# eldariont/svim

Measured on AMD Instinct MI355X. Metric: aligned reads/sec through COLLECT+CLUSTER, higher is better.
Workload: dtype u32/i32 CIGAR + u8 bases, int64 positions, f64 distances

## Files before the change

include/svx.h:

```cpp
#ifndef SVX_H
#define SVX_H
#include <stdint.h>
#ifdef __cplusplus
extern "C" {
#endif

#define SVX_OK               0
#define SVX_E_NODEVICE     (-1)
#define SVX_E_HIP          (-2)
#define SVX_E_ARG          (-3)
#define SVX_E_CAPACITY     (-4)
#define SVX_E_STATE        (-5)
#define SVX_E_FASTA_SYMBOL (-6)
#define SVX_E_FASTA_HOST   (-7)
#define SVX_E_NO_DELETION  (-8)

enum { SVX_DEL = 0, SVX_INS = 1, SVX_INV = 2, SVX_DUP_TAN = 3, SVX_BND = 4, SVX_DUP_INT = 5, SVX_NTYPES = 6 };
enum { SVX_SRC_CIGAR = 0, SVX_SRC_SUPPL = 1 };
enum { SVX_LEFT_FWD = 0, SVX_LEFT_REV = 1, SVX_RIGHT_FWD = 2, SVX_RIGHT_REV = 3, SVX_DIR_ALL = 4 };

#define SVX_FLAG_SKIP 0x8000u
#define SVX_FLAG_SA   0x4000u

typedef struct svx_params {
// ... 27 lines not shown
    const uint32_t* seg_off;
    int64_t n_seg;
    const int32_t*  seg_tid;
    const int32_t*  seg_pos;
    const uint8_t*  seg_rev;
    const uint8_t*  seg_mapq;
    const int32_t*  seg_lseq;
    const uint64_t* seg_cigar_off;
    const uint32_t* seg_cigar;
    int32_t n_contig;
    const int32_t*  contig_rank;
    const uint32_t* seq_rng_off;
    const int32_t*  seq_rng_q0;
    const int32_t*  seq_rng_len;
    const uint64_t* seq_rng_byte;
    int64_t n_seq_rng;
} svx_batch;

typedef struct svx_sig_view {
    int32_t on_device;
    int64_t n;
    uint64_t* key;
    uint8_t*  type;
    uint8_t*  src;
    uint8_t*  aux;
    int32_t*  contig;
    int32_t*  start;
    int32_t*  end;
    int32_t*  contig2;
    int32_t*  pos2;
    int32_t*  read_id;
    int64_t*  seq_off;
    uint8_t*  seq;
} svx_sig_view;

typedef struct svx_genome {
    int32_t on_device;
    int32_t n_contig;
    const int64_t* off;
    const uint8_t* codes;
} svx_genome;

typedef struct svx_cluster_view {
    int64_t n;
    int64_t type_count[SVX_NTYPES];
    uint8_t* type;
    int32_t* contig;  int32_t* start;  int32_t* end;
    int32_t* contig2; int32_t* start2; int32_t* end2;
    uint8_t* aux;
    double*  score;
    double*  std_span;
    double*  std_pos;
    int32_t* size;
    int64_t* member_off;
    int32_t* members;
    int64_t  n_members;
} svx_cluster_view;

typedef struct svx_ctx svx_ctx;

typedef struct svx_stats {
    double  t_collect_ms, t_cluster_ms;
    double  t_cigar_scan_ms, t_segments_ms, t_sort_ms, t_partition_ms, t_edit_ms, t_linkage_ms, t_gather_ms;
    int64_t n_rec_used, n_ops, n_seg, n_seg_ops, n_sig, n_bnd_side, n_ins_bases;
    int64_t n_partitions, n_large_partitions, n_pairs, n_edit_pairs, n_edit_cells, n_clusters, n_hap_bytes;
    int64_t n_edit_wordcols_issued, n_edit_wordcols_useful, n_edit_wordcols_retry, n_edit_wordcols_band;
    double  edit_guess;
} svx_stats;

int  svx_ctx_create(int device_ordinal, svx_ctx** out);
void svx_ctx_destroy(svx_ctx* ctx);
const char* svx_last_error(void);
int  svx_version(void);
int  svx_get_stats(svx_ctx* ctx, svx_stats* out);
void* svx_stream(svx_ctx* ctx);
int  svx_memcpy_d2h(void* host_dst, const void* device_src, uint64_t bytes);
int  svx_memcpy_h2d(void* device_dst, const void* host_src, uint64_t bytes);
void* svx_dev_alloc(uint64_t bytes);
void svx_dev_free(void* p);
void* svx_host_alloc(uint64_t bytes);
void svx_host_free(void* p);
int  svx_device_synchronize(void);
int  svx_selftest_prims(svx_ctx* ctx, int64_t n, int32_t begin_bit, int32_t end_bit, uint64_t seed);

int  svx_collect(svx_ctx* ctx, const svx_batch* batch, const svx_params* p);
int  svx_collect_accumulate(svx_ctx* ctx, int mode);
int  svx_collect_set_slot_base(svx_ctx* ctx, uint64_t slot_base);
int  svx_collect_count(svx_ctx* ctx, int64_t* n_sig, int64_t* n_seq_bytes, int64_t* n_bnd_side);
int  svx_collect_fetch(svx_ctx* ctx, int which, svx_sig_view* host_out);

#define SVX_FASTA_TILE        4096
#define SVX_FASTA_PIECE       (8 << 20)
#define SVX_FASTA_NAME_BYTES  256
enum { SVX_FASTA_PLAIN = 0, SVX_FASTA_BGZF = 1, SVX_FASTA_GZIP = 2 };
enum { SVX_FASTA_HOST_NONE = 0, SVX_FASTA_HOST_BLANKS = 1 ,
       SVX_FASTA_HOST_BUDGET = 2 ,
       SVX_FASTA_HOST_NAMES = 3 ,
       SVX_FASTA_HOST_CONTAINER = 4  };
typedef struct svx_fasta_stats {
    int32_t kind;
    int32_t host_reason;
    int64_t raw_bytes;
    int64_t seq_bytes;
    int64_t dropped_bytes;
    int64_t blank_bytes;
    int64_t bases_kept;
    int64_t records_in_file, records_kept;
    int64_t blocks;
    double  t_read_stage_s;
    double  t_inflate_s;
    double  t_kernels_s;
    double  t_total_s;
    uint32_t bad_mask[8];
} svx_fasta_stats;
int  svx_genome_load_fasta(svx_ctx* ctx, const char* path, int32_t n_contig, const char* names_nul_separated,
                           int64_t* off_out , svx_fasta_stats* stats );
int  svx_genome_fetch(svx_ctx* ctx, int32_t* n_contig, int64_t* n_codes, int64_t* off , uint8_t* codes );
int  svx_fasta_probe(const char* path, int32_t* kind, int64_t* raw_bytes, int64_t* n_blocks);
int  svx_fasta_plan(int64_t n_hdr, const uint8_t* name_blob, const int64_t* hdr_pos, const int64_t* hdr_rank, int64_t raw_bytes, int32_t n_contig,
                    const char* names_nul_separated, int64_t* dest, int64_t* off_out, int64_t* records_kept );

int  svx_set_genome(svx_ctx* ctx, const svx_genome* g);
int  svx_cluster(svx_ctx* ctx, int source, const svx_sig_view* sigs, int32_t n_contig,
                 const int32_t* contig_rank_host, const svx_params* p);
int  svx_cluster_count(svx_ctx* ctx, int64_t* n_clusters, int64_t* n_members);
int  svx_cluster_fetch(svx_ctx* ctx, svx_cluster_view* out);
int  svx_cluster_partitions_fetch(svx_ctx* c, int64_t* n_sig, int64_t* n_part, uint32_t* sorted_index, int64_t* part_start);

typedef int (*svx_allgather_fn)(void* user, const void* send, void* recv, int64_t bytes);
int  svx_cluster_set_ranks(svx_ctx* ctx, int rank, int world, svx_allgather_fn fn, void* user);
int  svx_cluster_abort_ranks(svx_ctx* ctx);
int  svx_cluster_stream_positions(svx_ctx* ctx, int64_t* start , int64_t* end );

typedef struct svx_combine_params {
    int64_t trans_sv_max_distance;
    double  del_ins_dup_max_distance;
    double  position_distance_normalizer;
    int64_t partition_max_distance;
    double  cluster_max_distance;
} svx_combine_params;
enum { SVX_CAND_DEL = 0, SVX_CAND_INV = 1, SVX_CAND_DUP_INT = 2, SVX_CAND_DUP_TAN = 3, SVX_CAND_INS = 4, SVX_CAND_BND = 5, SVX_NCAND = 6 };
typedef struct svx_candidate_view {
    int64_t n;
    int64_t n_members;
    int64_t class_count[SVX_NCAND];
    uint8_t* cls;
    int32_t* contig;  int32_t* start;  int32_t* end;
    int32_t* contig2; int32_t* start2; int32_t* end2;
    uint8_t* aux;
    int32_t* copies;
    double*  score;
    double*  std_span;
    double*  std_pos;
    int64_t* member_off;
    int32_t* members;
} svx_candidate_view;
typedef struct svx_combine_stats {
    double  t_combine_ms;
    double  t_cutpaste_ms;
    int64_t n_clusters_in, n_bnd_mirrored, n_merged, n_insertion_from, n_deletions, n_cutpaste_pairs, n_cutpaste;
    int64_t n_remove_1, n_remove_2, n_dup_partitions, n_dup_large_partitions, n_candidates, n_candidate_members;
} svx_combine_stats;
int  svx_combine(svx_ctx* ctx, int source, const svx_cluster_view* clusters, const uint8_t* sig_aux, int64_t n_sig, int32_t on_device, int32_t n_contig,
                 const int32_t* contig_rank_host, const svx_combine_params* p);
int  svx_combine_count(svx_ctx* ctx, int64_t* n_candidates, int64_t* n_members);
int  svx_combine_fetch(svx_ctx* ctx, svx_candidate_view* out);
// ... 60 lines not shown
```

svim_amd/_lib.py:

```python
import ctypes as C
import os
import subprocess

import numpy as np

from . import _abi
from ._abi import ClusterTable, SigTable, ptr

_HERE = os.path.dirname(os.path.abspath(__file__))
_LIB_PATH = os.environ.get("SVX_LIB") or os.path.join(_HERE, "libsvx.so")
_LIB = None
_ENGINES = {}

SYMBOLS = ["svx_ctx_create", "svx_ctx_destroy", "svx_last_error", "svx_version", "svx_get_stats", "svx_stream", "svx_cluster_partitions_fetch", "svx_memcpy_d2h", "svx_memcpy_h2d", "svx_dev_alloc", "svx_dev_free", "svx_host_alloc", "svx_host_free", "svx_device_synchronize", "svx_selftest_prims", "svx_bam_set_device_decode",
           "svx_collect", "svx_collect_count", "svx_collect_fetch", "svx_collect_accumulate", "svx_collect_set_slot_base", "svx_set_genome", "svx_cluster",
           "svx_cluster_count", "svx_cluster_fetch", "svx_cluster_set_ranks", "svx_cluster_abort_ranks", "svx_cluster_stream_positions",
           "svx_set_alignment_index", "svx_genotype",
           "svx_cigar_indel", "svx_edit_distance", "svx_linkage_fcluster", "svx_pair_distances",
           "svx_bam_open", "svx_bam_close", "svx_bam_header", "svx_bam_read_batch", "svx_bam_read_names", "svx_bam_set_seq_filter", "svx_bam_rewind", "svx_bam_seek", "svx_bam_set_gpu_inflate", "svx_bam_gpu_inflate_stats",
           "svx_inflater_create", "svx_inflater_destroy", "svx_inflater_staging", "svx_inflater_enqueue", "svx_inflater_wait",
           "svx_inflater_run",
           "svx_genome_load_fasta", "svx_genome_fetch", "svx_fasta_probe", "svx_fasta_plan",
           "svx_combine", "svx_combine_count", "svx_combine_fetch", "svx_combine_stages_fetch", "svx_combine_get_stats", "svx_py_sample100"]


class SvxError(RuntimeError):
    pass


class FastaHostRoute(SvxError):

    def __init__(self, msg, code, stats):
        SvxError.__init__(self, msg)
        self.code = code
        self.stats = stats


def _names_blob(references):
    names = [r.encode("utf-8") if isinstance(r, str) else bytes(r) for r in references]
    if any(b"\0" in n for n in names):
        raise ValueError("contig names must not contain NUL")
    return b"".join(n + b"\0" for n in names)


def fasta_probe(path):
    kind, raw, nb = C.c_int32(), C.c_int64(), C.c_int64()
    _check(lib().svx_fasta_probe(os.fsencode(path), C.byref(kind), C.byref(raw), C.byref(nb)), "svx_fasta_probe")
    return _abi.FASTA_KINDS[kind.value], raw.value, nb.value


def fasta_plan(name_blob, hdr_pos, hdr_rank, raw_bytes, references):
    hdr_pos = np.ascontiguousarray(hdr_pos, dtype=np.int64)
    hdr_rank = np.ascontiguousarray(hdr_rank, dtype=np.int64)
    n_hdr = int(hdr_pos.size)
    blob = np.frombuffer(bytes(name_blob), dtype=np.uint8) if n_hdr else np.zeros(1, np.uint8)
    if hdr_rank.size != n_hdr + 1 or (n_hdr and blob.size != n_hdr * _abi.FASTA_NAME_BYTES):
        raise ValueError("fasta_plan: hdr_rank needs n_hdr + 1 entries, name_blob n_hdr * %d bytes" % _abi.FASTA_NAME_BYTES)
    dest = np.zeros(max(1, n_hdr), dtype=np.int64)
    off = np.zeros(len(references) + 1, dtype=np.int64)
    kept = C.c_int64()
    rc = lib().svx_fasta_plan(C.c_int64(n_hdr), ptr(blob), ptr(hdr_pos if n_hdr else np.zeros(1, np.int64)), ptr(hdr_rank), C.c_int64(int(raw_bytes)),
                              C.c_int32(len(references)), _names_blob(references), ptr(dest), ptr(off), C.byref(kept))
    if rc == _abi.SVX_E_FASTA_HOST:
        raise FastaHostRoute(lib().svx_last_error().decode("utf-8", "replace"), rc, None)
    _check(rc, "svx_fasta_plan")
    return dest[:n_hdr], off, kept.value


class NoDeletionClusters(SvxError):
    """svx_combine met insertion-from clusters but no deletion cluster (SVX_E_NO_DELETION): the reference raises IndexError there
    (src/svim/SVIM_merging.py:20), and so does svim_amd.SVIM_COMBINE.combine_clusters"""


def py_sample100(sizes):
    sizes = np.ascontiguousarray(sizes, dtype=np.int64)
    out = np.zeros((max(1, sizes.size), 100), dtype=np.int32)
    _check(lib().svx_py_sample100(C.c_int64(sizes.size), ptr(sizes if sizes.size else np.zeros(1, np.int64)), ptr(out)), "svx_py_sample100")
    return out[:sizes.size]


def build(force=False):
    if force:
        subprocess.check_call(["make", "-s", "-C", os.path.join(_HERE, "csrc"), "clean"])
    subprocess.check_call(["make", "-s", "-j8", "-C", os.path.join(_HERE, "csrc")])
    return _LIB_PATH


def lib():
    global _LIB
    if _LIB is None:
        if not os.path.exists(_LIB_PATH):
            raise SvxError("svim_amd/libsvx.so is not built (run `python -c 'import __graft_entry__ as g; g.build()'` "
                           "or `make -C svim_amd/csrc`); the GPU path has no CPU fallback")
        L = C.CDLL(_LIB_PATH)
        L.svx_last_error.restype = C.c_char_p
        L.svx_stream.restype = C.c_void_p
        _LIB = L
# ... 140 lines not shown
        return self.fetch_candidates() if fetch else None

    def fetch_candidates(self):
        n, nm = C.c_int64(), C.c_int64()
        _check(self.L.svx_combine_count(self.ctx, C.byref(n), C.byref(nm)), "svx_combine_count")
        t = _abi.CandidateTable(n.value, nm.value)
        v = t.view()
        _check(self.L.svx_combine_fetch(self.ctx, C.byref(v)), "svx_combine_fetch")
        return t.finish(v)

    def combine_stages(self):
        mv, fv = _abi.CandidateView(), _abi.CandidateView()
        n1, n2 = C.c_int64(), C.c_int64()
        _check(self.L.svx_combine_stages_fetch(self.ctx, C.byref(mv), C.byref(n1), None, C.byref(n2), None, C.byref(fv)), "svx_combine_stages_fetch")
        merged, flagged = _abi.CandidateTable(mv.n, mv.n_members), _abi.CandidateTable(fv.n, fv.n_members)
        r1, r2 = np.zeros(max(1, n1.value), np.int32), np.zeros(max(1, n2.value), np.int32)
        mv, fv = merged.view(), flagged.view()
        _check(self.L.svx_combine_stages_fetch(self.ctx, C.byref(mv), C.byref(n1), ptr(r1), C.byref(n2), ptr(r2), C.byref(fv)), "svx_combine_stages_fetch")
        return {"merged": merged.finish(mv), "remove_1": r1[:n1.value], "remove_2": r2[:n2.value], "flagged": flagged.finish(fv)}

    def combine_stats(self):
        s = _abi.CombineStats()
        _check(self.L.svx_combine_get_stats(self.ctx, C.byref(s)), "svx_combine_get_stats")
        return s.as_dict()

    def set_alignment_index(self, index):
        v = index.view()
        _check(self.L.svx_set_alignment_index(self.ctx, C.byref(v)), "svx_set_alignment_index")

    def genotype(self, mode, tid, start, end, member_off, member_names, min_mapq):
        n = len(tid)
        out = np.zeros(max(1, n), dtype=np.int32)
        tid = np.ascontiguousarray(tid, dtype=np.int32); start = np.ascontiguousarray(start, dtype=np.int32)
        end = np.ascontiguousarray(end, dtype=np.int32); member_off = np.ascontiguousarray(member_off, dtype=np.int64)
        member_names = np.ascontiguousarray(member_names, dtype=np.int32)
        _check(self.L.svx_genotype(self.ctx, C.c_int32(mode), C.c_int64(n), ptr(tid), ptr(start), ptr(end), ptr(member_off),
                                   ptr(member_names if member_names.size else np.zeros(1, np.int32)), C.c_int32(min_mapq), ptr(out)), "svx_genotype")
        return out[:n]

    def set_ranks(self, rank, world, allgather=None):
        if allgather is None or world <= 1:
            self._ag_cb = None
            _check(self.L.svx_cluster_set_ranks(self.ctx, 0, 1, None, None), "svx_cluster_set_ranks")
            return
        proto = C.CFUNCTYPE(C.c_int, C.c_void_p, C.c_void_p, C.c_void_p, C.c_int64)

        into = getattr(allgather, "gather_into", None)

        def tramp(user, send, recv, nbytes):
            try:
                if into is not None and nbytes > 0:
                    into(int(send), int(recv), int(nbytes))
                    return 0
                got = allgather(C.string_at(send, nbytes))
                if len(got) != nbytes * world:
                    raise ValueError("all-gather callback returned %d bytes, expected %d" % (len(got), nbytes * world))
                C.memmove(recv, got, len(got))
                return 0
            except Exception:
                import traceback
                traceback.print_exc()
                return 1
        self._ag_cb = proto(tramp)
        _check(self.L.svx_cluster_set_ranks(self.ctx, int(rank), int(world), self._ag_cb, None), "svx_cluster_set_ranks")

    def abort_ranks(self):
        _check(self.L.svx_cluster_abort_ranks(self.ctx), "svx_cluster_abort_ranks")

    def stream_positions(self):
        a, b = (C.c_int64 * 6)(), (C.c_int64 * 6)()
        _check(self.L.svx_cluster_stream_positions(self.ctx, a, b), "svx_cluster_stream_positions")
        return list(a), list(b)

    def stats(self):
        s = _abi.Stats()
        _check(self.L.svx_get_stats(self.ctx, C.byref(s)), "svx_get_stats")
        return s.as_dict()

    def stream(self):
        return self.L.svx_stream(self.ctx)

    def selftest_prims(self, n, begin_bit=0, end_bit=64, seed=1):
        _check(self.L.svx_selftest_prims(self.ctx, C.c_int64(n), C.c_int32(begin_bit), C.c_int32(end_bit), C.c_uint64(seed)), "svx_selftest_prims")

    def cigar_indel(self, tuples, min_length):
        c = np.array([(l << 4) | op for op, l in tuples] or [0], dtype=np.uint32)
        n = len(tuples)
        o_ref = np.zeros(max(1, n), dtype=np.int64)
        o_read = np.zeros(max(1, n), dtype=np.int64)
        o_len = np.zeros(max(1, n), dtype=np.int32)
        o_del = np.zeros(max(1, n), dtype=np.uint8)
        m = C.c_int64()
        _check(self.L.svx_cigar_indel(self.ctx, ptr(c), C.c_int64(n), C.c_int32(min_length), ptr(o_ref), ptr(o_read),
                                      ptr(o_len), ptr(o_del), C.byref(m)), "svx_cigar_indel")
        return [(int(o_ref[i]), int(o_read[i]), int(o_len[i]), "DEL" if o_del[i] else "INS") for i in range(m.value)]

    def edit_distances(self, pairs):
        chunks, a_off, b_off = [], [0], [0]
        pos = 0
        for a, _ in pairs:
            c = _abi.encode_bases(a)
            chunks.append(c)
            pos += c.size
            a_off.append(pos)
        b_off = [pos]
        for _, b in pairs:
            c = _abi.encode_bases(b)
            chunks.append(c)
            pos += c.size
            b_off.append(pos)
        codes = np.concatenate(chunks + [np.zeros(1, np.uint8)])
        a_off = np.array(a_off, dtype=np.int64)
        b_off = np.array(b_off, dtype=np.int64)
        out = np.zeros(max(1, len(pairs)), dtype=np.int32)
        _check(self.L.svx_edit_distance(self.ctx, C.c_int64(len(pairs)), ptr(codes), ptr(a_off), ptr(b_off), ptr(out)),
               "svx_edit_distance")
        return [int(x) for x in out[:len(pairs)]]

    def pair_distances(self, table, pairs, params):
        ia = np.ascontiguousarray([i for i, _ in pairs], dtype=np.int64)
        ib = np.ascontiguousarray([j for _, j in pairs], dtype=np.int64)
        out = np.zeros(max(1, len(pairs)), dtype=np.float64)
        v = table.view()
        _check(self.L.svx_pair_distances(self.ctx, C.byref(v), C.c_int64(len(pairs)), ptr(ia), ptr(ib), C.byref(params), ptr(out)), "svx_pair_distances")
        return out[:len(pairs)]

    def linkage_fcluster(self, problems, cutoff):
        ns = np.array([p[0] for p in problems], dtype=np.int32)
        d_off = np.zeros(len(problems) + 1, dtype=np.int64)
        l_off = np.zeros(len(problems) + 1, dtype=np.int64)
        for i, (n, d) in enumerate(problems):
            d_off[i + 1] = d_off[i] + n * (n - 1) // 2
            l_off[i + 1] = l_off[i] + n
        d = np.concatenate([np.asarray(p[1], dtype=np.float64).ravel() for p in problems] + [np.zeros(1)])
        lab = np.zeros(max(1, int(l_off[-1])), dtype=np.int32)
        _check(self.L.svx_linkage_fcluster(self.ctx, C.c_int64(len(problems)), ptr(ns), ptr(d_off), ptr(d), C.c_double(cutoff),
                                           ptr(l_off), ptr(lab)), "svx_linkage_fcluster")
        return [lab[l_off[i]:l_off[i + 1]].copy() for i in range(len(problems))]


def engine(device=None):
    if device is None:
        device = int(os.environ.get("LOCAL_RANK", "0"))
    e = _ENGINES.get(device)
    if e is None:
        e = _ENGINES[device] = Engine(device)
    return e


def bgzf_blocks(path):
    import struct
    with open(path, "rb") as fh:
        data = fh.read()
    at, out = 0, []
    while at + 18 <= len(data):
        if data[at:at + 2] != b"\x1f\x8b":
            raise ValueError("not a BGZF block at %d" % at)
        xlen = struct.unpack_from("<H", data, at + 10)[0]
        p, bsize = at + 12, None
        while p + 4 <= at + 12 + xlen:
            si, sl = data[p:p + 2], struct.unpack_from("<H", data, p + 2)[0]
            if si == b"BC":
                bsize = struct.unpack_from("<H", data, p + 4)[0]
            p += 4 + sl
        if bsize is None:
            raise ValueError("no BC subfield")
# ... 48 lines not shown
```

svim_amd/csrc/common.hpp:

```cpp
#pragma once
#include <chrono>
#include <hip/hip_runtime.h>
#include <cstdint>
#include <cstdio>
#include <cstring>
#include <string>
#include <vector>
#include "../../include/svx.h"

#define SVX_FLAG_USED_MASK (SVX_FLAG_SKIP | 4u | 256u)

extern thread_local std::string g_svx_err;
int svx_fail(int code, const char* what, const char* file, int line, hipError_t e);

#define HIPCHK(expr)                                                                                   \
    do {                                                                                               \
        hipError_t e_ = (expr);                                                                        \
        if (e_ != hipSuccess) return svx_fail(SVX_E_HIP, #expr, __FILE__, __LINE__, e_);               \
    } while (0)
#define SVXCHK(expr)                                                                                   \
    do {                                                                                               \
        int rc_ = (expr);                                                                              \
        if (rc_ != SVX_OK) return rc_;                                                                 \
    } while (0)
// ... 29 lines not shown
        if (p) { if (svx_guard_mode()) svx_guard_free(p); else (void)hipFree(p); }
        p = nullptr;
        cap = 0;
    }
    template <class T> T* as() const { return reinterpret_cast<T*>(p); }
};

struct DevSigs {
    int64_t n = 0, cap = 0;
    DevBuf key, type, src, aux, contig, start, end, contig2, pos2, read_id, rec, qpos, qlen;
    DevBuf seq_off, seq;
    int64_t n_seq = 0;
    int reserve(int64_t c) {
        if (c <= cap) return SVX_OK;
        SVXCHK(key.reserve(c * 8)); SVXCHK(type.reserve(c)); SVXCHK(src.reserve(c)); SVXCHK(aux.reserve(c));
        SVXCHK(contig.reserve(c * 4)); SVXCHK(start.reserve(c * 4)); SVXCHK(end.reserve(c * 4));
        SVXCHK(contig2.reserve(c * 4)); SVXCHK(pos2.reserve(c * 4)); SVXCHK(read_id.reserve(c * 4));
        SVXCHK(rec.reserve(c * 4)); SVXCHK(qpos.reserve(c * 4)); SVXCHK(qlen.reserve(c * 4));
        cap = c;
        return SVX_OK;
    }
    int reserve_keep(int64_t c, hipStream_t s) {
        if (c <= cap) return SVX_OK;
        const int64_t nc = c + c / 2 + 1024;
        DevBuf* b8[] = {&key}; DevBuf* b1[] = {&type, &src, &aux}; DevBuf* b4[] = {&contig, &start, &end, &contig2, &pos2, &read_id};
        for (auto* b : b8) SVXCHK(b->reserve((size_t)nc * 8, true, s));
        for (auto* b : b1) SVXCHK(b->reserve((size_t)nc, true, s));
        for (auto* b : b4) SVXCHK(b->reserve((size_t)nc * 4, true, s));
        SVXCHK(seq_off.reserve((size_t)(nc + 2) * 8, true, s));
        cap = nc;
        return SVX_OK;
    }
    void release() {
        DevBuf* all[] = {&key, &type, &src, &aux, &contig, &start, &end, &contig2, &pos2, &read_id, &rec, &qpos, &qlen, &seq_off, &seq};
        for (auto* b : all) b->release();
        n = cap = 0;
    }
};

struct SigPtrs {
    uint64_t* key; uint8_t* type; uint8_t* src; uint8_t* aux;
    int32_t *contig, *start, *end, *contig2, *pos2, *read_id, *rec, *qpos, *qlen;
};
inline SigPtrs sig_ptrs(const DevSigs& d) {
    SigPtrs p;
    p.key = d.key.as<uint64_t>(); p.type = d.type.as<uint8_t>(); p.src = d.src.as<uint8_t>(); p.aux = d.aux.as<uint8_t>();
    p.contig = d.contig.as<int32_t>(); p.start = d.start.as<int32_t>(); p.end = d.end.as<int32_t>();
    p.contig2 = d.contig2.as<int32_t>(); p.pos2 = d.pos2.as<int32_t>(); p.read_id = d.read_id.as<int32_t>();
    p.rec = d.rec.as<int32_t>(); p.qpos = d.qpos.as<int32_t>(); p.qlen = d.qlen.as<int32_t>();
    return p;
}

struct ClusterIn {
    int64_t n;
    const uint8_t* type; const uint8_t* aux;
    const int32_t *contig, *start, *end, *contig2, *pos2, *read_id;
    const int64_t* seq_off; const uint8_t* seq;
};

struct DevClusters {
    int64_t n = 0, n_members = 0, cap = 0;
    int64_t type_count[SVX_NTYPES] = {0, 0, 0, 0, 0, 0};
    DevBuf type, contig, start, end, contig2, start2, end2, aux, score, std_span, std_pos, size, member_off, members, part_index;
};

#define SVX_N_AUX 8

struct svx_ctx {
    int device = 0;
    int n_cu = 256;
    hipStream_t stream = nullptr;
    hipEvent_t ev[24];
    hipStream_t aux[SVX_N_AUX];
    std::vector<DevBuf> batch_bufs;
    DevSigs sig, bnd;
    DevSigs acc_sig, acc_bnd; bool accumulate = false; uint64_t slot_base = 0;
    DevSigs raw_sig, raw_bnd;
    DevBuf counters;
    DevBuf shard_cnt;
    DevBuf raw_indel;
    DevBuf rec_geom, seg_geom;
    DevBuf seg_ws;
    DevBuf tmp0, tmp1, tmp2, tmp3, tmp4, tmp5, sort_tmp, scan_tmp;
    DevBuf g_off, g_codes; int32_t g_n = 0; bool g_borrowed = false; const int64_t* g_off_p = nullptr; const uint8_t* g_codes_p = nullptr;
    DevBuf user_sig[12]; DevBuf c_rank;
    DevBuf k_hi, k_lo, k_idx, k_hi2, k_lo2, k_idx2, part_flag, part_id, part_start, part_meta, samp_idx, large_list, samp_stream;
    DevBuf cell_shards;
    DevBuf geno[11]; int64_t geno_n = 0; int32_t geno_contigs = -1;
    DevBuf samp_meta, samp_table, samp_runs, samp_chain;
    int xr_rank = 0, xr_world = 1; svx_allgather_fn xr_fn = nullptr; void* xr_user = nullptr; bool xr_pending = false;
    long long stream_start[SVX_NTYPES] = {0, 0, 0, 0, 0, 0}, stream_end[SVX_NTYPES] = {0, 0, 0, 0, 0, 0};
    DevBuf mt_words; long long mt_have = 0;
    DevBuf pair_off, ed, work, stage, stage_members, labels;
    DevBuf e_words, e_off, e_scratch, e_rec, e_desc, e_key, e_val, e_slot, e_fail, e_big_list, e_big_state, e_big_off;
    DevBuf e_blk[2];
    DevBuf e_retry[3];
    DevClusters clu;
    float edit_guess = 0.125f; bool edit_guess_pinned = false; float edit_guess_last = 0.125f;
    int prepack_state = 0; long long prepack_radius = 0, prepack_n = 0; DevBuf prepack_tmp;
    int64_t* pinned = nullptr;
    unsigned long long* mail = nullptr; unsigned long long mail_seq = 0; int mail_mode = 1;
    DevBuf e_hist;
    bool edit_force_full = false;
    bool no_seq_gather = false;
    svx_stats stats;
    int64_t last_cluster_source_n = 0;
    const uint8_t* last_cluster_aux = nullptr; long long cluster_calls = 0;
    struct CombineState* combine = nullptr;
};
void svx_combine_release(svx_ctx* c);

int svx_sort_pairs_u64(svx_ctx* c, const uint64_t* keys_in, uint64_t* keys_out, const uint32_t* vals_in, uint32_t* vals_out,
                       int64_t n, int begin_bit, int end_bit);
int svx_exclusive_scan_i64(svx_ctx* c, const int64_t* in, int64_t* out, int64_t n);
int svx_exclusive_scan_i64_on(svx_ctx* c, const int64_t* in, int64_t* out, int64_t n, hipStream_t stream, DevBuf& tmp);
int svx_exclusive_scan_i32_to_i64(svx_ctx* c, const int32_t* in, int64_t* out, int64_t n);

#define SVX_MAIL_SLOTS 16
#define SVX_MAIL_WORDS 512
struct MailSrc { const void* p[4]; int n[4]; int k; };
int svx_mail_post(svx_ctx* c, hipStream_t st, const MailSrc& src, unsigned long long* ticket);
int svx_mail_wait(svx_ctx* c, hipStream_t st, unsigned long long ticket, const unsigned long long** payload);
inline int svx_mail_gather(svx_ctx* c, hipStream_t st, int k, const void* const* srcs, const int* n_words, void* const* dsts) {
    MailSrc m; memset(&m, 0, sizeof m);
    m.k = k;
    for (int j = 0; j < k; j++) { m.p[j] = srcs[j]; m.n[j] = n_words[j]; }
    unsigned long long t = 0; const unsigned long long* w = nullptr;
    SVXCHK(svx_mail_post(c, st, m, &t));
    SVXCHK(svx_mail_wait(c, st, t, &w));
    for (int j = 0; j < k; j++) { memcpy(dsts[j], w, (size_t)n_words[j] * 8); w += n_words[j]; }
    return SVX_OK;
}
inline int svx_mail_read(svx_ctx* c, hipStream_t st, const void* dev_src, int n_words, void* host_dst) {
    const void* srcs[1] = {dev_src}; const int n[1] = {n_words}; void* dsts[1] = {host_dst};
    return svx_mail_gather(c, st, 1, srcs, n, dsts);
}
inline int svx_mail_read2(svx_ctx* c, hipStream_t st, const void* a, int na, void* da, const void* b, int nb, void* db) {
    const void* srcs[2] = {a, b}; const int n[2] = {na, nb}; void* dsts[2] = {da, db};
    return svx_mail_gather(c, st, 2, srcs, n, dsts);
}
inline int svx_mail_read3(svx_ctx* c, hipStream_t st, const void* a, int na, void* da, const void* b, int nb, void* db, const void* e, int ne, void* de) {
    const void* srcs[3] = {a, b, e}; const int n[3] = {na, nb, ne}; void* dsts[3] = {da, db, de};
    return svx_mail_gather(c, st, 3, srcs, n, dsts);
}

void svx_preload_collect(); void svx_preload_cluster(); void svx_preload_edit(); void svx_preload_prims(); void svx_preload_combine();

int svx_collect_impl(svx_ctx* c, const svx_batch* b_dev, const svx_params* p);
int svx_cluster_impl(svx_ctx* c, const ClusterIn& in, int32_t n_contig, const int32_t* rank_dev, const svx_params* p);
void svx_exchange_poison(svx_ctx* c);
int svx_edit_prepack_begin(svx_ctx* c, const ClusterIn& in, const svx_params& p, hipEvent_t input_ready);
int svx_edit_prepack_pack(svx_ctx* c, const ClusterIn& in);
int svx_pair_distances_impl(svx_ctx* c, const ClusterIn& in, int64_t n_pairs, const int64_t* ia_dev, const int64_t* ib_dev, const svx_params* p, double* out_dev);
int svx_set_alignment_index_impl(svx_ctx* c, const svx_aln_index* h);
int svx_genotype_impl(svx_ctx* c, int32_t mode, int64_t n_cand, const int32_t* tid, const int32_t* start, const int32_t* end, const int64_t* moff,
                      const int32_t* mnames, int32_t min_mapq, int32_t* out);
int svx_edit_distance_pairs(svx_ctx* c, int64_t n_pairs, const uint8_t* codes_dev, const int64_t* a_off_dev, const int64_t* b_off_dev, int32_t* out_dev);
int svx_linkage_batch(svx_ctx* c, int64_t n_problems, const int32_t* n_dev, const int64_t* d_off_dev, const double* d_dev, double cutoff,
                      const int64_t* label_off_dev, int32_t* labels_dev);

#ifdef __HIPCC__
__device__ __forceinline__ int lane_id() { return (int)(threadIdx.x & 63); }
__device__ __forceinline__ uint64_t lanemask_lt() { return (1ull << lane_id()) - 1ull; }

#define SVX_DPP_ADD(dst_, src_, ctrl_, row_, bank_) dst_ += __builtin_amdgcn_update_dpp(0, src_, ctrl_, row_, bank_, true)
__device__ __forceinline__ int wave_incl_scan_i32(int v) {
// ... 53 lines not shown
```

svim_amd/csrc/prims.hip:

```cpp
#include "common.hpp"
#include "scan.hpp"
#include "hostcopy.hpp"
#include <algorithm>
#include <vector>

#define RADIX_T 256
#define RADIX_ITEMS 8
#define RADIX_TILE (RADIX_T * RADIX_ITEMS)
#define RADIX_ONE_T 1024
#define RADIX_ONE (2 * RADIX_ONE_T * RADIX_ITEMS)

__device__ __forceinline__ unsigned radix_digit(uint64_t key, int shift, unsigned mask) { return (unsigned)(key >> shift) & mask; }

__device__ __forceinline__ void radix_rank_tile(const unsigned (&dig)[RADIX_ITEMS], unsigned (*wh_)[256], unsigned (&rank)[RADIX_ITEMS]) {
    const int w = (int)(threadIdx.x >> 6), lane = lane_id();
    volatile unsigned* wh = wh_[w];
    for (int d = lane; d < 256; d += 64) wh[d] = 0;
    __builtin_amdgcn_wave_barrier();
#pragma unroll
    for (int r = 0; r < RADIX_ITEMS; r++) {
        const unsigned d = dig[r];
        const bool live = d < 256u;
        unsigned long long peers = __ballot(live);
#pragma unroll
        for (int b = 0; b < 8; b++) {
            const unsigned long long m = __ballot((d >> b) & 1u);
            peers &= ((d >> b) & 1u) ? m : ~m;
        }
        const unsigned below = (unsigned)__popcll(peers & lanemask_lt()), cnt = (unsigned)__popcll(peers);
        const int leader = peers ? __ffsll((long long)peers) - 1 : 0;
        unsigned old = 0;
        if (live && lane == leader) { old = wh[d]; wh[d] = old + cnt; }
        old = (unsigned)__shfl((int)old, leader, 64);
        rank[r] = old + below;
        __builtin_amdgcn_wave_barrier();
    }
}

__global__ __launch_bounds__(RADIX_T) void k_radix_hist(const uint64_t* keys, long long n, int shift, unsigned mask, long long tiles, unsigned* cnt, unsigned* digit_total) {
    __shared__ unsigned h[256];
    h[threadIdx.x] = 0;
    __syncthreads();
    const long long lo = (long long)blockIdx.x * RADIX_TILE;
#pragma unroll
    for (int k = 0; k < RADIX_ITEMS; k++) {
        const long long i = lo + (long long)k * RADIX_T + threadIdx.x;
        if (i < n) atomicAdd(&h[radix_digit(keys[i], shift, mask)], 1u);
    }
    __syncthreads();
    const unsigned v = h[threadIdx.x];
    cnt[(long long)threadIdx.x * tiles + blockIdx.x] = v;
    if (v) atomicAdd(digit_total + threadIdx.x, v);
}

__global__ __launch_bounds__(256) void k_radix_offsets(const unsigned* cnt, const unsigned* digit_total, long long tiles, unsigned* off) {
    __shared__ unsigned sh[256 / 64 + 1];
    const int d = (int)blockIdx.x;
    unsigned total;
    unsigned carry;
    {
        const unsigned mine = (int)threadIdx.x < d ? digit_total[threadIdx.x] : 0u;
        (void)scan_block_excl<unsigned>(mine, sh, &total);
        carry = total;
    }
    const unsigned* c = cnt + (long long)d * tiles;
    unsigned* o = off + (long long)d * tiles;
    for (long long lo = 0; lo < tiles; lo += 256) {
        const long long t = lo + threadIdx.x;
        const unsigned mine = t < tiles ? c[t] : 0u;
        const unsigned ex = scan_block_excl<unsigned>(mine, sh, &total);
        if (t < tiles) o[t] = carry + ex;
        carry += total;
    }
}

__global__ __launch_bounds__(RADIX_T) void k_radix_scatter(const uint64_t* keys_in, const uint32_t* vals_in, uint64_t* keys_out, uint32_t* vals_out, long long n, int shift,
                                                           unsigned mask, long long tiles, const unsigned* off) {
    __shared__ unsigned wh[RADIX_T / 64][256];
    __shared__ unsigned base[RADIX_T / 64][256];
    const int w = (int)(threadIdx.x >> 6), lane = lane_id();
    const long long lo = (long long)blockIdx.x * RADIX_TILE + (long long)w * (64 * RADIX_ITEMS);
    uint64_t key[RADIX_ITEMS]; uint32_t val[RADIX_ITEMS]; unsigned dig[RADIX_ITEMS], rank[RADIX_ITEMS];
#pragma unroll
    for (int r = 0; r < RADIX_ITEMS; r++) {
        const long long i = lo + (long long)r * 64 + lane;
        key[r] = i < n ? keys_in[i] : 0ull;
        val[r] = i < n ? vals_in[i] : 0u;
        dig[r] = i < n ? radix_digit(key[r], shift, mask) : 256u;
    }
    radix_rank_tile(dig, wh, rank);
    __syncthreads();
    {
        const int d = (int)threadIdx.x;
        unsigned at = off[(long long)d * tiles + blockIdx.x];
#pragma unroll
        for (int k = 0; k < RADIX_T / 64; k++) { base[k][d] = at; at += wh[k][d]; }
    }
    __syncthreads();
#pragma unroll
    for (int r = 0; r < RADIX_ITEMS; r++) {
        if (dig[r] < 256u) {
            const unsigned p = base[w][dig[r]] + rank[r];
            keys_out[p] = key[r];
            vals_out[p] = val[r];
        }
    }
}

__global__ __launch_bounds__(RADIX_ONE_T) void k_radix_one(const uint64_t* keys_in, const uint32_t* vals_in, uint64_t* keys_out, uint32_t* vals_out, uint64_t* ktmp, uint32_t* vtmp,
                                                           long long n, int begin_bit, int end_bit) {
    __shared__ unsigned wh[RADIX_ONE_T / 64][256];
    __shared__ unsigned base[RADIX_ONE_T / 64][256];
    __shared__ unsigned tot[256];
    __shared__ unsigned sh[RADIX_ONE_T / 64 + 1];
    __shared__ unsigned n_used;
    const int w = (int)(threadIdx.x >> 6), lane = lane_id();
    const int passes = (end_bit - begin_bit + 7) / 8;
    const long long trip = (long long)RADIX_ONE_T * RADIX_ITEMS;
    const uint64_t* ks = keys_in; const uint32_t* vs = vals_in;
    uint64_t* kd = keys_out; uint32_t* vd = vals_out;
    for (int p = 0; p < passes; p++) {
        const int shift = begin_bit + 8 * p;
        const int bits = end_bit - shift < 8 ? end_bit - shift : 8;
        const unsigned mask = (1u << bits) - 1u;
        if (threadIdx.x < 256) tot[threadIdx.x] = 0;
        if (threadIdx.x == 0) n_used = 0;
        __syncthreads();
        for (long long i = threadIdx.x; i < n; i += RADIX_ONE_T) atomicAdd(&tot[radix_digit(ks[i], shift, mask)], 1u);
        __syncthreads();
        if (threadIdx.x < 256 && tot[threadIdx.x]) atomicAdd(&n_used, 1u);
        unsigned total;
        const unsigned start = scan_block_excl<unsigned, RADIX_ONE_T>(threadIdx.x < 256 ? tot[threadIdx.x] : 0u, sh, &total);
        __syncthreads();
        if (n_used <= 1u) continue;
        if (threadIdx.x < 256) tot[threadIdx.x] = start;
        __syncthreads();
        for (long long t0 = 0; t0 < n; t0 += trip) {
            const long long lo = t0 + (long long)w * (64 * RADIX_ITEMS);
            uint64_t key[RADIX_ITEMS]; uint32_t val[RADIX_ITEMS]; unsigned dig[RADIX_ITEMS], rank[RADIX_ITEMS];
#pragma unroll
            for (int r = 0; r < RADIX_ITEMS; r++) {
                const long long i = lo + (long long)r * 64 + lane;
                key[r] = i < n ? ks[i] : 0ull;
                val[r] = i < n ? vs[i] : 0u;
                dig[r] = i < n ? radix_digit(key[r], shift, mask) : 256u;
            }
            radix_rank_tile(dig, wh, rank);
            __syncthreads();
            if (threadIdx.x < 256) {
                const int d = (int)threadIdx.x;
                unsigned at = tot[d];
#pragma unroll
                for (int k = 0; k < RADIX_ONE_T / 64; k++) { base[k][d] = at; at += wh[k][d]; }
                tot[d] = at;
            }
            __syncthreads();
#pragma unroll
            for (int r = 0; r < RADIX_ITEMS; r++) {
                if (dig[r] < 256u) {
                    const unsigned q = base[w][dig[r]] + rank[r];
                    kd[q] = key[r];
                    vd[q] = val[r];
                }
            }
            __syncthreads();
        }
        __threadfence();
        __syncthreads();
        ks = kd; vs = vd;
        kd = kd == keys_out ? ktmp : keys_out; vd = vd == vals_out ? vtmp : vals_out;
    }
    if (ks != keys_out)
        for (long long i = threadIdx.x; i < n; i += RADIX_ONE_T) { keys_out[i] = ks[i]; vals_out[i] = vs[i]; }
}

int svx_sort_pairs_u64(svx_ctx* c, const uint64_t* keys_in, uint64_t* keys_out, const uint32_t* vals_in, uint32_t* vals_out,
                       int64_t n, int begin_bit, int end_bit) {
    if (n <= 0) return SVX_OK;
    if (n >= (1ll << 32) || begin_bit < 0 || end_bit > 64 || begin_bit >= end_bit) return svx_fail(SVX_E_ARG, "svx_sort_pairs_u64: bad arguments", __FILE__, __LINE__, hipSuccess);
    hipStream_t st = c->stream;
    const int passes = (end_bit - begin_bit + 7) / 8;
    const long long tiles = (n + RADIX_TILE - 1) / RADIX_TILE;
    const size_t pair_bytes = ((size_t)n * 8 + 255) / 256 * 256, val_bytes = ((size_t)n * 4 + 255) / 256 * 256;
    const size_t table = ((size_t)256 * (size_t)tiles * 4 + 255) / 256 * 256, totals = (size_t)passes * 256 * 4;
    SVXCHK(c->sort_tmp.reserve(pair_bytes + val_bytes + 2 * table + totals + 256));
    uint8_t* base = c->sort_tmp.as<uint8_t>();
    uint64_t* ktmp = reinterpret_cast<uint64_t*>(base);
    uint32_t* vtmp = reinterpret_cast<uint32_t*>(base + pair_bytes);
    if (n <= RADIX_ONE) {
        k_radix_one<<<1, RADIX_ONE_T, 0, st>>>(keys_in, vals_in, keys_out, vals_out, ktmp, vtmp, n, begin_bit, end_bit);
        HIPCHK(hipGetLastError());
        return SVX_OK;
    }
    unsigned* cnt = reinterpret_cast<unsigned*>(base + pair_bytes + val_bytes);
    unsigned* off = reinterpret_cast<unsigned*>(base + pair_bytes + val_bytes + table);
    unsigned* digit_total = reinterpret_cast<unsigned*>(base + pair_bytes + val_bytes + 2 * table);
    HIPCHK(hipMemsetAsync(digit_total, 0, totals, st));
    const uint64_t* ks = keys_in; const uint32_t* vs = vals_in;
    for (int p = 0; p < passes; p++) {
        const int shift = begin_bit + 8 * p;
        const int bits = end_bit - shift < 8 ? end_bit - shift : 8;
        const unsigned mask = (1u << bits) - 1u;
        uint64_t* kd = ((passes - 1 - p) & 1) ? ktmp : keys_out;
        uint32_t* vd = ((passes - 1 - p) & 1) ? vtmp : vals_out;
        k_radix_hist<<<(unsigned)tiles, RADIX_T, 0, st>>>(ks, n, shift, mask, tiles, cnt, digit_total + 256 * p);
        k_radix_offsets<<<256, 256, 0, st>>>(cnt, digit_total + 256 * p, tiles, off);
        k_radix_scatter<<<(unsigned)tiles, RADIX_T, 0, st>>>(ks, vs, kd, vd, n, shift, mask, tiles, off);
        ks = kd; vs = vd;
    }
    HIPCHK(hipGetLastError());
    return SVX_OK;
}

int svx_exclusive_scan_i64(svx_ctx* c, const int64_t* in, int64_t* out, int64_t n) {
    return svx_exclusive_scan<int64_t, int64_t>(in, out, n, c->stream, c->scan_tmp);
}
int svx_exclusive_scan_i64_on(svx_ctx* c, const int64_t* in, int64_t* out, int64_t n, hipStream_t stream, DevBuf& tmp) {
    (void)c;
    return svx_exclusive_scan<int64_t, int64_t>(in, out, n, stream, tmp);
}
int svx_exclusive_scan_i32_to_i64(svx_ctx* c, const int32_t* in, int64_t* out, int64_t n) {
    return svx_exclusive_scan<int32_t, int64_t>(in, out, n, c->stream, c->scan_tmp);
}

extern "C" int svx_selftest_prims(svx_ctx* c, int64_t n, int32_t begin_bit, int32_t end_bit, uint64_t seed) {
    if (!c || n < 0) return svx_fail(SVX_E_ARG, "bad argument", __FILE__, __LINE__, hipSuccess);
    HIPCHK(hipSetDevice(c->device));
    std::vector<uint64_t> k((size_t)n), k2((size_t)n);
    std::vector<uint32_t> v((size_t)n), v2((size_t)n);
    std::vector<int64_t> s((size_t)n + 1), s2((size_t)n + 1);
    uint64_t x = seed | 1ull;
    auto rnd = [&]() { x ^= x << 13; x ^= x >> 7; x ^= x << 17; return x; };
    for (int64_t i = 0; i < n; i++) {
        const uint64_t r = rnd();
        k[(size_t)i] = (r & 1) ? r : (r >> 40);
        if ((r & 6) == 0) k[(size_t)i] &= 0xffull << begin_bit;
        if (seed & 0x100) k[(size_t)i] &= 0xffff00ull;
        v[(size_t)i] = (uint32_t)i;
        s[(size_t)i] = (int64_t)(rnd() % 1000) - 100;
    }
    s[(size_t)n] = 0;
    DevBuf dk, dk2, dv, dv2, ds, ds2;
    auto done = [&](int r) { dk.release(); dk2.release(); dv.release(); dv2.release(); ds.release(); ds2.release(); return r; };
    auto on_device = [&]() -> int {
        SVXCHK(dk.reserve((size_t)n * 8 + 8)); SVXCHK(dk2.reserve((size_t)n * 8 + 8)); SVXCHK(dv.reserve((size_t)n * 4 + 8)); SVXCHK(dv2.reserve((size_t)n * 4 + 8));
        SVXCHK(ds.reserve((size_t)(n + 1) * 8)); SVXCHK(ds2.reserve((size_t)(n + 1) * 8));
        if (n) {
            SVXCHK(svx_h2d(dk.p, k.data(), (size_t)n * 8, c->stream));
            SVXCHK(svx_h2d(dv.p, v.data(), (size_t)n * 4, c->stream));
        }
        SVXCHK(svx_h2d(ds.p, s.data(), (size_t)(n + 1) * 8, c->stream));
        SVXCHK(svx_sort_pairs_u64(c, dk.as<uint64_t>(), dk2.as<uint64_t>(), dv.as<uint32_t>(), dv2.as<uint32_t>(), n, begin_bit, end_bit));
        SVXCHK(svx_exclusive_scan_i64(c, ds.as<int64_t>(), ds2.as<int64_t>(), n + 1));
        HIPCHK(hipStreamSynchronize(c->stream));
        if (n) {
            SVXCHK(svx_d2h(k2.data(), dk2.p, (size_t)n * 8, c->stream));
            SVXCHK(svx_d2h(v2.data(), dv2.p, (size_t)n * 4, c->stream));
        }
        SVXCHK(svx_d2h(s2.data(), ds2.p, (size_t)(n + 1) * 8, c->stream));
        return SVX_OK;
    };
    const int rc = on_device();
    if (rc != SVX_OK) return done(rc);
    const uint64_t m = (end_bit - begin_bit >= 64 ? ~0ull : ((1ull << (end_bit - begin_bit)) - 1ull)) << begin_bit;
    std::vector<uint32_t> order((size_t)n);
    for (int64_t i = 0; i < n; i++) order[(size_t)i] = (uint32_t)i;
    std::stable_sort(order.begin(), order.end(), [&](uint32_t a, uint32_t b) { return (k[a] & m) < (k[b] & m); });
    for (int64_t i = 0; i < n; i++)
        if (v2[(size_t)i] != order[(size_t)i] || k2[(size_t)i] != k[order[(size_t)i]]) return done(svx_fail(SVX_E_STATE, "radix sort differs from std::stable_sort", __FILE__, __LINE__, hipSuccess));
    int64_t run = 0;
    for (int64_t i = 0; i <= n; i++) {
        if (s2[(size_t)i] != run) return done(svx_fail(SVX_E_STATE, "exclusive scan differs from the serial sum", __FILE__, __LINE__, hipSuccess));
        run += s[(size_t)i];
    }
    return done(SVX_OK);
}

void svx_preload_prims() { hipFuncAttributes a; (void)hipFuncGetAttributes(&a, reinterpret_cast<const void*>(&k_radix_offsets)); (void)hipGetLastError(); }
```

Measured before the change: 70.96 million.

## Add onesweep radix sort with decoupled look-back and skipped uniform passes

Adds a onesweep-style LSD radix sort. A single histogram kernel computes the digit counts for every pass at once. A plan kernel then skips passes whose digit is uniform across all keys. Each scatter pass uses a hierarchical decoupled look-back (tile and group descriptors) in place of separate offset/scan kernels. This path is on by default for sorts with more than three passes, and an env var can turn it off. It aims to cut kernel launches and global memory passes over the keys, but it relies on forward-progress spinning that is only caught by an error flag, which is checked only in the self-test and host-test paths.

```diff
diff --git a/include/svx.h b/include/svx.h
--- a/include/svx.h
+++ b/include/svx.h
@@ -133,6 +133,7 @@
 void svx_host_free(void* p);
 int  svx_device_synchronize(void);
 int  svx_selftest_prims(svx_ctx* ctx, int64_t n, int32_t begin_bit, int32_t end_bit, uint64_t seed);
+int  svx_sort_pairs_host(svx_ctx* ctx, const uint64_t* keys, int64_t n, int32_t begin_bit, int32_t end_bit, int32_t mode, uint64_t* keys_out, uint32_t* order_out);
 
 int  svx_collect(svx_ctx* ctx, const svx_batch* batch, const svx_params* p);
 int  svx_collect_accumulate(svx_ctx* ctx, int mode);
diff --git a/svim_amd/_lib.py b/svim_amd/_lib.py
--- a/svim_amd/_lib.py
+++ b/svim_amd/_lib.py
@@ -12,7 +12,7 @@
 _LIB = None
 _ENGINES = {}
 
-SYMBOLS = ["svx_ctx_create", "svx_ctx_destroy", "svx_last_error", "svx_version", "svx_get_stats", "svx_stream", "svx_cluster_partitions_fetch", "svx_memcpy_d2h", "svx_memcpy_h2d", "svx_dev_alloc", "svx_dev_free", "svx_host_alloc", "svx_host_free", "svx_device_synchronize", "svx_selftest_prims", "svx_bam_set_device_decode",
+SYMBOLS = ["svx_ctx_create", "svx_ctx_destroy", "svx_last_error", "svx_version", "svx_get_stats", "svx_stream", "svx_cluster_partitions_fetch", "svx_memcpy_d2h", "svx_memcpy_h2d", "svx_dev_alloc", "svx_dev_free", "svx_host_alloc", "svx_host_free", "svx_device_synchronize", "svx_selftest_prims", "svx_sort_pairs_host", "svx_bam_set_device_decode",
            "svx_collect", "svx_collect_count", "svx_collect_fetch", "svx_collect_accumulate", "svx_collect_set_slot_base", "svx_set_genome", "svx_cluster",
            "svx_cluster_count", "svx_cluster_fetch", "svx_cluster_set_ranks", "svx_cluster_abort_ranks", "svx_cluster_stream_positions",
            "svx_set_alignment_index", "svx_genotype",
@@ -319,6 +319,13 @@
 
     def selftest_prims(self, n, begin_bit=0, end_bit=64, seed=1):
         _check(self.L.svx_selftest_prims(self.ctx, C.c_int64(n), C.c_int32(begin_bit), C.c_int32(end_bit), C.c_uint64(seed)), "svx_selftest_prims")
+
+    def sort_pairs(self, keys, begin_bit=0, end_bit=64, mode=-1):
+        keys = np.ascontiguousarray(keys, dtype=np.uint64)
+        out, order = np.empty_like(keys), np.empty(keys.shape[0], dtype=np.uint32)
+        _check(self.L.svx_sort_pairs_host(self.ctx, keys.ctypes.data_as(C.c_void_p), C.c_int64(keys.shape[0]), C.c_int32(begin_bit), C.c_int32(end_bit),
+                                          C.c_int32(mode), out.ctypes.data_as(C.c_void_p), order.ctypes.data_as(C.c_void_p)), "svx_sort_pairs_host")
+        return out, order
 
     def cigar_indel(self, tuples, min_length):
         c = np.array([(l << 4) | op for op, l in tuples] or [0], dtype=np.uint32)
diff --git a/svim_amd/csrc/common.hpp b/svim_amd/csrc/common.hpp
--- a/svim_amd/csrc/common.hpp
+++ b/svim_amd/csrc/common.hpp
@@ -135,6 +135,8 @@
     DevBuf rec_geom, seg_geom;
     DevBuf seg_ws;
     DevBuf tmp0, tmp1, tmp2, tmp3, tmp4, tmp5, sort_tmp, scan_tmp;
+    int sort_mode = -1;
+    void* sort_last_ctl = nullptr;
     DevBuf g_off, g_codes; int32_t g_n = 0; bool g_borrowed = false; const int64_t* g_off_p = nullptr; const uint8_t* g_codes_p = nullptr;
     DevBuf user_sig[12]; DevBuf c_rank;
     DevBuf k_hi, k_lo, k_idx, k_hi2, k_lo2, k_idx2, part_flag, part_id, part_start, part_meta, samp_idx, large_list, samp_stream;
diff --git a/svim_amd/csrc/prims.hip b/svim_amd/csrc/prims.hip
--- a/svim_amd/csrc/prims.hip
+++ b/svim_amd/csrc/prims.hip
@@ -2,6 +2,7 @@
 #include "scan.hpp"
 #include "hostcopy.hpp"
 #include <algorithm>
+#include <cstdlib>
 #include <vector>
 
 #define RADIX_T 256
@@ -103,6 +104,162 @@
             const unsigned p = base[w][dig[r]] + rank[r];
             keys_out[p] = key[r];
             vals_out[p] = val[r];
+        }
+    }
+}
+
+#define RADIX_MAX_PASSES 8
+#define RADIX_LOOK 8
+#define RADIX_ST_SHIFT 30
+#define RADIX_PUBLISHED (1u << 31)
+#define RADIX_VAL_MASK ((1u << RADIX_ST_SHIFT) - 1u)
+#define RADIX_GROUP_MIN 32
+#define RADIX_SPIN_LIMIT (1u << 24)
+#define RADIX_HIST_GRID 256
+
+struct RadixCtl {
+    unsigned total[RADIX_MAX_PASSES][256];
+    unsigned start[RADIX_MAX_PASSES][256];
+    unsigned ticket[RADIX_MAX_PASSES];
+    unsigned plan[RADIX_MAX_PASSES];
+    unsigned error;
+};
+
+__global__ __launch_bounds__(RADIX_T) void k_radix_hist_all(const uint64_t* keys, long long n, int begin_bit, int end_bit, int passes, long long tiles, RadixCtl* ctl,
+                                                            unsigned* desc0, long long desc_words) {
+    __shared__ unsigned h[RADIX_MAX_PASSES][256];
+    const int lane = lane_id();
+    for (int p = 0; p < passes; p++) h[p][threadIdx.x] = 0;
+    __syncthreads();
+    for (long long i = (long long)blockIdx.x * RADIX_T + threadIdx.x; i < desc_words; i += (long long)gridDim.x * RADIX_T) desc0[i] = 0;
+    for (long long tile = blockIdx.x; tile < tiles; tile += gridDim.x) {
+        const long long lo = tile * RADIX_TILE;
+#pragma unroll
+        for (int k = 0; k < RADIX_ITEMS; k++) {
+            const long long i = lo + (long long)k * RADIX_T + threadIdx.x;
+            const bool live = i < n;
+            const uint64_t key = live ? keys[i] : 0ull;
+            const unsigned long long lv = __ballot(live);
+            if (!lv) continue;
+            for (int p = 0; p < passes; p++) {
+                const int shift = begin_bit + 8 * p;
+                const unsigned mask = (1u << (end_bit - shift < 8 ? end_bit - shift : 8)) - 1u;
+                const unsigned d = radix_digit(key, shift, mask);
+                const unsigned d0 = (unsigned)__builtin_amdgcn_readfirstlane((int)d);
+                if (__ballot(live && d == d0) == lv) { if (lane == 0) atomicAdd(&h[p][d0], (unsigned)__popcll(lv)); }
+                else if (live) atomicAdd(&h[p][d], 1u);
+            }
+        }
+    }
+    __syncthreads();
+    for (int p = 0; p < passes; p++) { const unsigned v = h[p][threadIdx.x]; if (v) atomicAdd(&ctl->total[p][threadIdx.x], v); }
+}
+
+__global__ __launch_bounds__(RADIX_T) void k_radix_plan(int passes, RadixCtl* ctl) {
+    __shared__ unsigned sh[RADIX_T / 64 + 1];
+    __shared__ unsigned s_active[RADIX_MAX_PASSES];
+    for (int p = 0; p < passes; p++) {
+        const unsigned v = ctl->total[p][threadIdx.x];
+        const int used = __syncthreads_count(v != 0u);
+        unsigned total;
+        ctl->start[p][threadIdx.x] = scan_block_excl<unsigned>(v, sh, &total);
+        if (threadIdx.x == 0) s_active[p] = used > 1 ? 1u : 0u;
+    }
+    __syncthreads();
+    if (threadIdx.x == 0) {
+        int act = 0;
+        for (int p = 0; p < passes; p++) act += (int)s_active[p];
+        if (!act) { s_active[passes - 1] = 1; act = 1; }
+        unsigned src = 0; int j = 0;
+        for (int p = 0; p < passes; p++) {
+            if (!s_active[p]) { ctl->plan[p] = 0; continue; }
+            const unsigned dst = ((act - 1 - j) & 1) ? 2u : 1u;
+            ctl->plan[p] = 1u | (src << 1) | (dst << 3) | ((unsigned)(j & 1) << 5);
+            src = dst; j++;
+        }
+    }
+}
+
+__device__ __forceinline__ unsigned radix_wait_sum(const unsigned* table, long long lo, long long hi, int d, unsigned* error) {
+    unsigned sum = 0, spins = 0;
+    long long r = lo;
+    while (r < hi) {
+        unsigned v[RADIX_LOOK];
+#pragma unroll
+        for (int k = 0; k < RADIX_LOOK; k++)
+            v[k] = r + k < hi ? __hip_atomic_load(table + (r + k) * 256 + d, __ATOMIC_RELAXED, __HIP_MEMORY_SCOPE_AGENT) : RADIX_PUBLISHED;
+        int used = 0;
+        bool open = true;
+#pragma unroll
+        for (int k = 0; k < RADIX_LOOK; k++) {
+            open = open && (v[k] & RADIX_PUBLISHED);
+            if (open) { sum += v[k] & RADIX_VAL_MASK; used++; }
+        }
+        r += used;
+        if (used == 0) {
+            __builtin_amdgcn_s_sleep(1);
+            if (++spins > RADIX_SPIN_LIMIT) { *error = 1u; break; }
+        }
+    }
+    return sum;
+}
+
+__global__ __launch_bounds__(RADIX_T) void k_radix_sweep(const uint64_t* keys_in, const uint32_t* vals_in, uint64_t* keys_out, uint32_t* vals_out, uint64_t* ktmp, uint32_t* vtmp,
+                                                         long long n, int p, int shift, unsigned mask, long long tiles, long long group, RadixCtl* ctl, unsigned* desc) {
+    const unsigned plan = ctl->plan[p];
+    if (!(plan & 1u)) return;
+    __shared__ unsigned wh[RADIX_T / 64][256];
+    __shared__ unsigned base[RADIX_T / 64][256];
+    __shared__ unsigned s_tile;
+    if (threadIdx.x == 0) s_tile = atomicAdd(&ctl->ticket[p], 1u);
+    __syncthreads();
+    const long long tile = (long long)s_tile;
+    const unsigned src = (plan >> 1) & 3u, dst = (plan >> 3) & 3u, tab = (plan >> 5) & 1u;
+    const uint64_t* ks = src == 0 ? keys_in : (src == 1 ? keys_out : ktmp);
+    const uint32_t* vs = src == 0 ? vals_in : (src == 1 ? vals_out : vtmp);
+    uint64_t* kd = dst == 1 ? keys_out : ktmp;
+    uint32_t* vd = dst == 1 ? vals_out : vtmp;
+    const long long groups = (tiles + group - 1) / group, table_words = (tiles + groups) * 256;
+    const long long g = tile / group, g_lo = g * group, g_hi = g_lo + group < tiles ? g_lo + group : tiles;
+    unsigned* rows = desc + (long long)tab * table_words;
+    unsigned* grows = rows + tiles * 256;
+    {
+        unsigned* next = desc + (long long)(tab ^ 1u) * table_words;
+        next[tile * 256 + threadIdx.x] = 0;
+        if (tile == g_lo) next[(tiles + g) * 256 + threadIdx.x] = 0;
+    }
+    const int w = (int)(threadIdx.x >> 6), lane = lane_id();
+    const long long lo = tile * RADIX_TILE + (long long)w * (64 * RADIX_ITEMS);
+    uint64_t key[RADIX_ITEMS]; uint32_t val[RADIX_ITEMS]; unsigned dig[RADIX_ITEMS], rank[RADIX_ITEMS];
+#pragma unroll
+    for (int r = 0; r < RADIX_ITEMS; r++) {
+        const long long i = lo + (long long)r * 64 + lane;
+        key[r] = i < n ? ks[i] : 0ull;
+        val[r] = i < n ? vs[i] : 0u;
+        dig[r] = i < n ? radix_digit(key[r], shift, mask) : 256u;
+    }
+    radix_rank_tile(dig, wh, rank);
+    __syncthreads();
+    {
+        const int d = (int)threadIdx.x;
+        unsigned cnt = 0;
+#pragma unroll
+        for (int k = 0; k < RADIX_T / 64; k++) cnt += wh[k][d];
+        __hip_atomic_store(rows + tile * 256 + d, RADIX_PUBLISHED | cnt, __ATOMIC_RELAXED, __HIP_MEMORY_SCOPE_AGENT);
+        unsigned before = radix_wait_sum(rows, g_lo, tile, d, &ctl->error);
+        if (tile == g_hi - 1) __hip_atomic_store(grows + g * 256 + d, RADIX_PUBLISHED | (before + cnt), __ATOMIC_RELAXED, __HIP_MEMORY_SCOPE_AGENT);
+        before += radix_wait_sum(grows, 0, g, d, &ctl->error);
+        unsigned at = ctl->start[p][d] + before;
+#pragma unroll
+        for (int k = 0; k < RADIX_T / 64; k++) { base[k][d] = at; at += wh[k][d]; }
+    }
+    __syncthreads();
+#pragma unroll
+    for (int r = 0; r < RADIX_ITEMS; r++) {
+        if (dig[r] < 256u) {
+            const unsigned q = base[w][dig[r]] + rank[r];
+            kd[q] = key[r];
+            vd[q] = val[r];
         }
     }
 }
@@ -174,6 +331,11 @@
         for (long long i = threadIdx.x; i < n; i += RADIX_ONE_T) { keys_out[i] = ks[i]; vals_out[i] = vs[i]; }
 }
 
+static bool sort_onesweep(const svx_ctx* c, int passes) {
+    static const bool env = []() { const char* e = getenv("SVX_SORT_ONESWEEP"); return !(e && e[0] == '0'); }();
+    return c->sort_mode < 0 ? env && passes > 3 : c->sort_mode != 0;
+}
+
 int svx_sort_pairs_u64(svx_ctx* c, const uint64_t* keys_in, uint64_t* keys_out, const uint32_t* vals_in, uint32_t* vals_out,
                        int64_t n, int begin_bit, int end_bit) {
     if (n <= 0) return SVX_OK;
@@ -182,6 +344,30 @@
     const int passes = (end_bit - begin_bit + 7) / 8;
     const long long tiles = (n + RADIX_TILE - 1) / RADIX_TILE;
     const size_t pair_bytes = ((size_t)n * 8 + 255) / 256 * 256, val_bytes = ((size_t)n * 4 + 255) / 256 * 256;
+    c->sort_last_ctl = nullptr;
+    if (n > RADIX_ONE && n < (1ll << RADIX_ST_SHIFT) && sort_onesweep(c, passes)) {
+        long long group = RADIX_GROUP_MIN;
+        while (group * group < tiles) group *= 2;
+        const long long groups = (tiles + group - 1) / group;
+        const size_t ctl_bytes = (sizeof(RadixCtl) + 255) / 256 * 256, table = (size_t)(tiles + groups) * 256 * 4;
+        SVXCHK(c->sort_tmp.reserve(pair_bytes + val_bytes + ctl_bytes + 2 * table + 256));
+        uint8_t* base = c->sort_tmp.as<uint8_t>();
+        uint64_t* ktmp = reinterpret_cast<uint64_t*>(base);
+        uint32_t* vtmp = reinterpret_cast<uint32_t*>(base + pair_bytes);
+        RadixCtl* ctl = reinterpret_cast<RadixCtl*>(base + pair_bytes + val_bytes);
+        unsigned* desc = reinterpret_cast<unsigned*>(base + pair_bytes + val_bytes + ctl_bytes);
+        HIPCHK(hipMemsetAsync(ctl, 0, sizeof(RadixCtl), st));
+        k_radix_hist_all<<<(unsigned)std::min<long long>(tiles, RADIX_HIST_GRID), RADIX_T, 0, st>>>(keys_in, n, begin_bit, end_bit, passes, tiles, ctl, desc, (tiles + groups) * 256);
+        k_radix_plan<<<1, RADIX_T, 0, st>>>(passes, ctl);
+        for (int p = 0; p < passes; p++) {
+            const int shift = begin_bit + 8 * p;
+            const int bits = end_bit - shift < 8 ? end_bit - shift : 8;
+            k_radix_sweep<<<(unsigned)tiles, RADIX_T, 0, st>>>(keys_in, vals_in, keys_out, vals_out, ktmp, vtmp, n, p, shift, (1u << bits) - 1u, tiles, group, ctl, desc);
+        }
+        HIPCHK(hipGetLastError());
+        c->sort_last_ctl = ctl;
+        return SVX_OK;
+    }
     const size_t table = ((size_t)256 * (size_t)tiles * 4 + 255) / 256 * 256, totals = (size_t)passes * 256 * 4;
     SVXCHK(c->sort_tmp.reserve(pair_bytes + val_bytes + 2 * table + totals + 256));
     uint8_t* base = c->sort_tmp.as<uint8_t>();
@@ -212,6 +398,13 @@
     return SVX_OK;
 }
 
+static int sort_check_last(svx_ctx* c) {
+    if (!c->sort_last_ctl) return SVX_OK;
+    unsigned err = 0;
+    SVXCHK(svx_d2h(&err, &static_cast<RadixCtl*>(c->sort_last_ctl)->error, 4, c->stream));
+    return err ? svx_fail(SVX_E_STATE, "radix sort: a look-back waited in vain for a tile before it", __FILE__, __LINE__, hipSuccess) : SVX_OK;
+}
+
 int svx_exclusive_scan_i64(svx_ctx* c, const int64_t* in, int64_t* out, int64_t n) {
     return svx_exclusive_scan<int64_t, int64_t>(in, out, n, c->stream, c->scan_tmp);
 }
@@ -253,6 +446,7 @@
         SVXCHK(svx_sort_pairs_u64(c, dk.as<uint64_t>(), dk2.as<uint64_t>(), dv.as<uint32_t>(), dv2.as<uint32_t>(), n, begin_bit, end_bit));
         SVXCHK(svx_exclusive_scan_i64(c, ds.as<int64_t>(), ds2.as<int64_t>(), n + 1));
         HIPCHK(hipStreamSynchronize(c->stream));
+        SVXCHK(sort_check_last(c));
         if (n) {
             SVXCHK(svx_d2h(k2.data(), dk2.p, (size_t)n * 8, c->stream));
             SVXCHK(svx_d2h(v2.data(), dv2.p, (size_t)n * 4, c->stream));
@@ -276,4 +470,30 @@
     return done(SVX_OK);
 }
 
+extern "C" int svx_sort_pairs_host(svx_ctx* c, const uint64_t* keys, int64_t n, int32_t begin_bit, int32_t end_bit, int32_t mode, uint64_t* keys_out, uint32_t* order_out) {
+    if (!c || n < 0 || (n && (!keys || !keys_out || !order_out))) return svx_fail(SVX_E_ARG, "bad argument", __FILE__, __LINE__, hipSuccess);
+    if (n == 0) return SVX_OK;
+    HIPCHK(hipSetDevice(c->device));
+    std::vector<uint32_t> v((size_t)n);
+    for (int64_t i = 0; i < n; i++) v[(size_t)i] = (uint32_t)i;
+    DevBuf dk, dk2, dv, dv2;
+    auto on_device = [&]() -> int {
+        SVXCHK(dk.reserve((size_t)n * 8 + 8)); SVXCHK(dk2.reserve((size_t)n * 8 + 8)); SVXCHK(dv.reserve((size_t)n * 4 + 8)); SVXCHK(dv2.reserve((size_t)n * 4 + 8));
+        SVXCHK(svx_h2d(dk.p, keys, (size_t)n * 8, c->stream));
+        SVXCHK(svx_h2d(dv.p, v.data(), (size_t)n * 4, c->stream));
+        c->sort_mode = mode;
+        const int rc = svx_sort_pairs_u64(c, dk.as<uint64_t>(), dk2.as<uint64_t>(), dv.as<uint32_t>(), dv2.as<uint32_t>(), n, begin_bit, end_bit);
+        c->sort_mode = -1;
+        SVXCHK(rc);
+        HIPCHK(hipStreamSynchronize(c->stream));
+        SVXCHK(sort_check_last(c));
+        SVXCHK(svx_d2h(keys_out, dk2.p, (size_t)n * 8, c->stream));
+        SVXCHK(svx_d2h(order_out, dv2.p, (size_t)n * 4, c->stream));
+        return SVX_OK;
+    };
+    const int rc = on_device();
+    dk.release(); dk2.release(); dv.release(); dv2.release();
+    return rc;
+}
+
 void svx_preload_prims() { hipFuncAttributes a; (void)hipFuncGetAttributes(&a, reinterpret_cast<const void*>(&k_radix_offsets)); (void)hipGetLastError(); }
```

Result: faster. 71.79 million, median of 6 (+1.2%).
